# facebookresearch/detectron2

Measured on NVIDIA H100. Metric: Mask R-CNN R50-FPN training hot-path images/sec (custom-op path fwd+bwd, 2 images/GPU), higher is better.
Workload: dtype f32

## Files before the change

### detectron2_b200/csrc/deform_conv_tc.cu

```cuda
#include <algorithm>
#include <cstdlib>

#include "common.cuh"
#include "tc_common.cuh"

using namespace d2b_tc;

namespace {

constexpr int kWorkerWarps = 16;
constexpr int kWorkers = kWorkerWarps * 32;
constexpr int kThreads = kWorkers + 128;
constexpr int kLaunchRegs = (65536 / kThreads) & ~7;
constexpr int kWorkerRegs = 112, kSideRegs = 24;
static_assert(kWorkers * kWorkerRegs + (kThreads - kWorkers) * kSideRegs <= kThreads * kLaunchRegs,
              "register budget exceeds the launch allocation");
constexpr int kMaxBN = 128;
constexpr int kRowsPerHalf = 128 / (2 * kWorkerWarps);
constexpr int kTile = 16384;
constexpr int kMaxSmem = 227 * 1024;
constexpr int kGcolPitch = 132;

struct TC {
  int N, Cin, H, W, Cout, kh, kw, sh, sw, ph, pw, dh, dw, G, DG, Ho, Wo, cpg, opg, cpdg, KK, HoWo;
  int pack, SG, cps, ops, cbs, U;
  int tiles_img;
  int stages_img;
  int MC;
  int nks;
  long long off_bs, mask_bs;
  int mask_sigmoid;
};

struct Epi {
  const float* scale;
  const float* shift;
  int relu;
};

struct K1P { int BN, noct, nkp, ksplit, S, tap_bytes, stage_bytes, red; };
struct K2P { int mper, msplit, tap_bytes; };
struct K3P { int BN, noct, sper, nsplit, S, stage_bytes; };

inline size_t align256(size_t v) { return (v + 255) & ~(size_t)255; }

bool make_tc(const d2b_dcn_params* p, TC& d) {
  if (!p) return false;
  d.N = p->N; d.Cin = p->Cin; d.H = p->H; d.W = p->W; d.Cout = p->Cout; d.kh = p->kh; d.kw = p->kw;
  d.sh = p->stride_h; d.sw = p->stride_w; d.ph = p->pad_h; d.pw = p->pad_w; d.dh = p->dil_h; d.dw = p->dil_w;
  d.G = p->groups; d.DG = p->deformable_groups;
  if (d.N < 0 || d.Cin <= 0 || d.H <= 0 || d.W <= 0 || d.Cout <= 0 || d.kh <= 0 || d.kw <= 0 || d.sh <= 0 || d.sw <= 0 ||
      d.ph < 0 || d.pw < 0 || d.dh <= 0 || d.dw <= 0 || d.G <= 0 || d.DG <= 0)
    return false;
  if (d.Cin % d.G || d.Cout % d.G || d.Cin % d.DG) return false;
  d.Ho = (d.H + 2 * d.ph - (d.dh * (d.kh - 1) + 1)) / d.sh + 1;
  d.Wo = (d.W + 2 * d.pw - (d.dw * (d.kw - 1) + 1)) / d.sw + 1;
  if (d.Ho <= 0 || d.Wo <= 0) return false;
  d.cpg = d.Cin / d.G; d.opg = d.Cout / d.G; d.cpdg = d.Cin / d.DG; d.KK = d.kh * d.kw; d.HoWo = d.Ho * d.Wo;
  if (d.cpg >= 64) {
    if (d.cpg % 64) return false;
    d.pack = 1;
  } else {
    if (d.cpg != 16 && d.cpg != 32) return false;
    d.pack = 64 / d.cpg;
    if (d.G % d.pack) return false;
  }
  if (d.cpdg % 64) return false;
  d.SG = d.G / d.pack; d.cps = d.cpg * d.pack; d.ops = d.opg * d.pack; d.cbs = d.cps / 64; d.U = d.KK * d.cbs;
  if (d.ops % 16) return false;
  if (d.KK > 49) return false;
  if ((long long)d.H * d.W * d.Cin >= (1LL << 29)) return false;
  if ((long long)d.HoWo * d.Cout >= (1LL << 31) || (long long)d.Cout * d.cpg * d.KK >= (1LL << 31)) return false;
  d.tiles_img = d2b_cdiv(d.HoWo, 128);
  d.stages_img = d2b_cdiv(d.HoWo, 64);
  d.MC = (d.U + 1) / 2;
  d.nks = d.ops / 64;
  if ((long long)d.N * d.tiles_img > 0x7fffffffLL) return false;
  d.off_bs = (long long)d.DG * 2 * d.KK * d.HoWo;
  d.mask_bs = (long long)d.DG * d.KK * d.HoWo;
  d.mask_sigmoid = 0;
  return true;
}

const float* use_fused_offset_mask(TC& d, const float* offset_mask) {
  d.off_bs = d.mask_bs = (long long)d.DG * 3 * d.KK * d.HoWo;
  d.mask_sigmoid = 1;
  return offset_mask + (size_t)d.DG * 2 * d.KK * d.HoWo;
}

int largest_tile(int n) {
  for (int t = kMaxBN; t >= 16; t >>= 1)
    if (n % t == 0) return t;
  return 0;
}

int best_split(long long base, int work, int max_split, int overhead) {
  int best = 1;
  long long best_cost = -1;
  for (int s = 1; s <= max_split; ++s) {
    const int per = d2b_cdiv(work, s);
    const int parts = d2b_cdiv(work, per);
    const long long cost = (long long)d2b_cdiv(base * parts, d2b_num_sms()) * (per + overhead);
    if (best_cost < 0 || cost < best_cost) {
      best_cost = cost;
      best = parts;
    }
  }
  return best;
}

bool plan_k1(const TC& d, K1P& k) {
  k.BN = largest_tile(d.ops);
  if (k.BN < 16) return false;
  k.noct = d.ops / k.BN;
  const int base = d.N * d.tiles_img * d.SG * k.noct;
  k.ksplit = best_split(base, d.KK, d.KK, 1);
  k.nkp = d2b_cdiv(d.KK, k.ksplit);
  k.ksplit = d2b_cdiv(d.KK, k.nkp);
  k.red = k.ksplit > 1;
  const int ndg = d.DG == 1 ? 1 : std::min(d.DG, d2b_cdiv(d.cps, d.cpdg) + 1);
  k.tap_bytes = ndg * k.nkp * 128 * 16;
  k.stage_bytes = 2 * kTile + 2 * k.BN * 128;
  k.S = 3;
  while (k.S > 1 && k.S * k.stage_bytes + k.tap_bytes + 1024 + 128 > kMaxSmem) --k.S;
  return k.S >= 2;
}

bool plan_k2(const TC& d, K2P& k) {
  if (d.ops % 64) return false;
  const int base = d.N * d.tiles_img * d.SG;
  k.msplit = best_split(base, d.MC, d.MC, 1);
  k.mper = d2b_cdiv(d.MC, k.msplit);
  k.msplit = d2b_cdiv(d.MC, k.mper);
  const int nkp = std::min(d.KK, (2 * k.mper + d.cbs - 1) / d.cbs + 1);
  const int ndg = d.DG == 1 ? 1 : std::min(d.DG, d2b_cdiv(d.cps, d.cpdg) + 1);
  k.tap_bytes = ndg * nkp * 128 * 16;
  return 2 * 4 * kTile + 128 * kGcolPitch * 4 + k.tap_bytes + 1024 + 128 <= kMaxSmem;
}

bool plan_k3(const TC& d, K3P& k) {
  if (d.ops % 64) return false;
  k.BN = largest_tile(d.ops);
  k.noct = d.ops / k.BN;
  const int units = d.MC * d.SG * k.noct;
  const int total = d.N * d.stages_img;
  k.nsplit = best_split(units, total, std::min(total, 4 * d2b_num_sms()), 3);
  k.sper = d2b_cdiv(total, k.nsplit);
  k.nsplit = d2b_cdiv(total, k.sper);
  k.stage_bytes = 2 * kTile + 2 * k.BN * 128;
  k.S = 3;
  while (k.S > 1 && k.S * k.stage_bytes + 4096 + 1024 + 128 > kMaxSmem) --k.S;
  return k.S >= 2;
}

struct TapRaw {
  float oh, ow, m;
};

__device__ __forceinline__ TapRaw tap_loads(const TC& d, const float* __restrict__ offset, const float* __restrict__ mask,
                                            int b, int dg, int kp, int p) {
  TapRaw r = {0.f, 0.f, 1.f};
  if (p < d.HoWo) {
    const size_t ob = (size_t)b * d.off_bs + ((size_t)dg * 2 * d.KK) * d.HoWo;
    r.oh = __ldg(offset + ob + (size_t)(2 * kp) * d.HoWo + p);
    r.ow = __ldg(offset + ob + (size_t)(2 * kp + 1) * d.HoWo + p);
    if (mask) r.m = __ldg(mask + (size_t)b * d.mask_bs + ((size_t)dg * d.KK + kp) * d.HoWo + p);
  }
  return r;
}

__device__ __forceinline__ int4 tap_finish(const TC& d, const TapRaw& r, bool has_mask, int kp, int p) {
  int4 t = make_int4(0, 0, 0, 0);
  if (p < d.HoWo) {
    const int ho = p / d.Wo, wo = p - ho * d.Wo;
    const int ki = kp / d.kw, kj = kp - ki * d.kw;
    const float hf = (float)(ho * d.sh - d.ph + ki * d.dh) + r.oh;
    const float wf = (float)(wo * d.sw - d.pw + kj * d.dw) + r.ow;
    float m = r.m;
    if (has_mask && d.mask_sigmoid) m = 1.f / (1.f + expf(-m));
    if (hf > -1.f && wf > -1.f && hf < (float)d.H && wf < (float)d.W) {
      const float hfl = floorf(hf), wfl = floorf(wf);
      const int hl = (int)hfl, wl = (int)wfl;
      const bool t0 = hl >= 0, t1 = hl + 1 <= d.H - 1, l0 = wl >= 0, l1 = wl + 1 <= d.W - 1;
      const int flags = (t0 && l0 ? 1 : 0) | (t0 && l1 ? 2 : 0) | (t1 && l0 ? 4 : 0) | (t1 && l1 ? 8 : 0);
      t.x = ((hl * d.W + wl + d.W + 1) << 4) | flags;
      t.y = __float_as_int(hf - hfl);
      t.z = __float_as_int(wf - wfl);
      t.w = __float_as_int(m);
    }
  }
  return t;
}

__device__ __forceinline__ int4 make_tap(const TC& d, const float* __restrict__ offset, const float* __restrict__ mask,
                                         int b, int dg, int kp, int p) {
  return tap_finish(d, tap_loads(d, offset, mask, b, dg, kp, p), mask != nullptr, kp, p);
}

struct Taps4 {
  float4 v0, v1, v2, v3;
};

__device__ __forceinline__ void load_corners(const float* __restrict__ xcb, uint32_t Cin, uint32_t rs, int code, Taps4& t) {
  const float* __restrict__ p = xcb + (uint32_t)(code >> 4) * Cin;
  const float4 z = make_float4(0.f, 0.f, 0.f, 0.f);
  t.v0 = (code & 1) ? __ldg(reinterpret_cast<const float4*>(p)) : z;
  t.v1 = (code & 2) ? __ldg(reinterpret_cast<const float4*>(p + Cin)) : z;
  t.v2 = (code & 4) ? __ldg(reinterpret_cast<const float4*>(p + rs)) : z;
  t.v3 = (code & 8) ? __ldg(reinterpret_cast<const float4*>(p + (rs + Cin))) : z;
}

__device__ __forceinline__ void interp4(const Taps4& t, float w0, float w1, float w2, float w3, float (&v)[4]) {
  const F2 z = f2_pack(0.f, 0.f), p0 = f2_pack(w0, w0), p1 = f2_pack(w1, w1), p2 = f2_pack(w2, w2), p3 = f2_pack(w3, w3);
  F2 a = f2_fma(p0, f2_pack(t.v0.x, t.v0.y), z), b = f2_fma(p0, f2_pack(t.v0.z, t.v0.w), z);
  a = f2_fma(p1, f2_pack(t.v1.x, t.v1.y), a);
  b = f2_fma(p1, f2_pack(t.v1.z, t.v1.w), b);
  a = f2_fma(p2, f2_pack(t.v2.x, t.v2.y), a);
  b = f2_fma(p2, f2_pack(t.v2.z, t.v2.w), b);
  a = f2_fma(p3, f2_pack(t.v3.x, t.v3.y), a);
  b = f2_fma(p3, f2_pack(t.v3.z, t.v3.w), b);
  f2_unpack(a, v[0], v[1]);
  f2_unpack(b, v[2], v[3]);
}

__device__ __forceinline__ void gather_store(const Taps4& t, int4 tap, uint8_t* a_hi, uint8_t* a_lo, uint32_t off,
                                             bool split) {
  const float lh = __int_as_float(tap.y), lw = __int_as_float(tap.z), m = __int_as_float(tap.w);
  const float hh = 1.f - lh, hw = 1.f - lw;
  float v[4];
  interp4(t, hh * hw * m, hh * lw * m, lh * hw * m, lh * lw * m, v);
  uint2 hi, lo;
  split4(v, hi, lo);
  *reinterpret_cast<uint2*>(a_hi + off) = hi;
  if (split) *reinterpret_cast<uint2*>(a_lo + off) = lo;
}

template <int BN, int kTransA, int kSplit>
__device__ __forceinline__ void mma_stage_(float (&acc)[BN / 4], uint32_t a_hi, uint32_t a_lo, uint32_t b_hi, uint32_t b_lo) {
  const int g = (threadIdx.x >> 7);
  const uint32_t ao = kTransA ? (uint32_t)(g & 1) * 8192u : (uint32_t)(g & 1) * 64u * 128u;
  const uint32_t bo = (uint32_t)(g >> 1) * (uint32_t)(BN / 2) * 128u;
  const uint32_t lbo = kTransA ? 8192u : 0u;
  wgmma_fence();
#pragma unroll
  for (int kk = 0; kk < 4; ++kk) {
    const uint32_t ak = ao + (kTransA ? (uint32_t)kk * 2048u : (uint32_t)kk * 32u), bk = bo + (uint32_t)kk * 32u;
    Wgmma<BN / 2, kTransA>::mma(acc, wgmma_desc(a_hi + ak, lbo, 1024), wgmma_desc(b_hi + bk, 0, 1024), 1);
    if (kSplit) {
      Wgmma<BN / 2, kTransA>::mma(acc, wgmma_desc(a_hi + ak, lbo, 1024), wgmma_desc(b_lo + bk, 0, 1024), 1);
      Wgmma<BN / 2, kTransA>::mma(acc, wgmma_desc(a_lo + ak, lbo, 1024), wgmma_desc(b_hi + bk, 0, 1024), 1);
    }
  }
  wgmma_commit();
}
template <int BN, int kTransA>
__device__ __forceinline__ void mma_stage(float (&acc)[BN / 4], uint32_t a_hi, uint32_t a_lo, uint32_t b_hi, uint32_t b_lo,
                                          int split) {
  if (split) mma_stage_<BN, kTransA, 1>(acc, a_hi, a_lo, b_hi, b_lo);
  else mma_stage_<BN, kTransA, 0>(acc, a_hi, a_lo, b_hi, b_lo);
}

template <int BN>
__device__ __forceinline__ int acc_row(int i) {
  const int t = threadIdx.x & 127;
  return (threadIdx.x >> 7 & 1) * 64 + (t >> 5) * 16 + ((t & 31) >> 2) + ((i >> 1) & 1) * 8;
}
template <int BN>
__device__ __forceinline__ int acc_col(int i) {
  return (threadIdx.x >> 8) * (BN / 2) + (i >> 2) * 8 + (threadIdx.x & 3) * 2 + (i & 1);
}

template <int BN>
__global__ void __launch_bounds__(kThreads, 1) dcn_fwd_tc_kernel(const float* __restrict__ xh,
                                                                   const float* __restrict__ offset,
                                                                   const float* __restrict__ mask,
                                                                   const uint8_t* __restrict__ wt, const Epi ep, const TC d,
                                                                   const K1P k, const int split, float* __restrict__ out,
                                                                   uint8_t* __restrict__ cols) {
  extern __shared__ uint8_t smem_raw[];
  uint8_t* smem = smem_raw + ((1024u - (smem_u32(smem_raw) & 1023u)) & 1023u);
  int4* taps = reinterpret_cast<int4*>(smem + k.S * k.stage_bytes);
  uint64_t* bars = reinterpret_cast<uint64_t*>(reinterpret_cast<uint8_t*>(taps) + k.tap_bytes);
  uint64_t* full_bar = bars;
  uint64_t* empty_bar = bars + k.S;

  const int tid = threadIdx.x, warp = tid >> 5, lane = tid & 31;
  const int b = blockIdx.x / d.tiles_img, p0 = (blockIdx.x - b * d.tiles_img) * 128;
  const int sg = blockIdx.y / k.noct, oct = blockIdx.y - sg * k.noct;
  const int kp0 = blockIdx.z * k.nkp, nkp = min(d.KK, kp0 + k.nkp) - kp0;
  const int nt = nkp * d.cbs;
  const int dg0 = (sg * d.cps) / d.cpdg;
  const bool saving = cols != nullptr && oct == 0;

  if (tid == 0) {
    for (int s = 0; s < k.S; ++s) {
      mbar_init(&full_bar[s], kWorkerWarps + 1);
      mbar_init(&empty_bar[s], kWorkerWarps + (saving ? 1 : 0));
    }
    mbar_init_fence();
  }
  if (tid < kWorkers) {
    const int ndg = ((sg + 1) * d.cps - 1) / d.cpdg - dg0 + 1;
    for (int i = tid; i < ndg * nkp * 128; i += kWorkers) {
      const int row = i & 127, r = i >> 7;
      const int dgl = r / nkp, kpl = r - dgl * nkp;
      taps[i] = make_tap(d, offset, mask, b, dg0 + dgl, kp0 + kpl, p0 + row);
    }
  }
  __syncthreads();
  if (warp < kWorkerWarps) reg_alloc<kWorkerRegs>();
  else reg_dealloc<kSideRegs>();

  if (warp < kWorkerWarps) {
    const int half = lane >> 4, q = lane & 15;
    const float* __restrict__ ximg = xh + (size_t)b * d.H * d.W * d.Cin - (size_t)(d.W + 1) * d.Cin;
    const uint32_t ucin = (uint32_t)d.Cin, urs = (uint32_t)(d.W * d.Cin);
    float acc[BN / 4];
#pragma unroll
    for (int i = 0; i < BN / 4; ++i) acc[i] = 0.f;
    int kpl = 0, cb = 0;
    auto stage = [&](int t) {
      const int s = t % k.S;
      const uint32_t par = (uint32_t)((t / k.S) & 1);
      const int cbase = sg * d.cps + cb * 64;
      const int4* __restrict__ tp = taps + ((cbase / d.cpdg - dg0) * nkp + kpl) * 128;
      const float* __restrict__ xc = ximg + cbase + q * 4;
      uint8_t* a_hi = smem + s * k.stage_bytes;
      uint8_t* a_lo = a_hi + kTile;
      mbar_wait(&empty_bar[s], par ^ 1u);
      {
        int4 tap[kRowsPerHalf];
        Taps4 c[kRowsPerHalf];
#pragma unroll
        for (int j = 0; j < kRowsPerHalf; ++j) tap[j] = tp[warp * 2 * kRowsPerHalf + j * 2 + half];
#pragma unroll
        for (int j = 0; j < kRowsPerHalf; ++j) load_corners(xc, ucin, urs, tap[j].x, c[j]);
#pragma unroll
        for (int j = 0; j < kRowsPerHalf; ++j) {
          const uint32_t r = (uint32_t)(warp * 2 * kRowsPerHalf + j * 2 + half);
          gather_store(c[j], tap[j], a_hi, a_lo, swz128(r, (uint32_t)(q >> 1)) + (uint32_t)(q & 1) * 8u, split != 0);
        }
      }
      fence_proxy_async();
      __syncwarp();
      if (lane == 0) mbar_arrive(&full_bar[s]);
      mbar_wait(&full_bar[s], par);
      const uint32_t sa = smem_u32(a_hi), sb = sa + 2 * kTile;
      mma_stage<BN, 0>(acc, sa, sa + kTile, sb, sb + (uint32_t)BN * 128u, split);
      if (++cb == d.cbs) { cb = 0; ++kpl; }
    };
    stage(0);
    for (int t = 1; t < nt; ++t) {
      stage(t);
      wgmma_wait<1>();
      __syncwarp();
      if (lane == 0) mbar_arrive(&empty_bar[(t - 1) % k.S]);
    }
    wgmma_wait<0>();
    const int oc0 = sg * d.ops + oct * k.BN;
    const bool add_shift = ep.shift != nullptr && blockIdx.z == 0;
#pragma unroll
    for (int i = 0; i < BN / 4; ++i) {
      const int p = p0 + acc_row<BN>(i);
      if (p >= d.HoWo) continue;
      const int oc = oc0 + acc_col<BN>(i);
      float* dst = out + ((size_t)b * d.Cout + oc) * d.HoWo + p;
      float v = acc[i];
      if (k.red) {
        red_add(dst, v + ((add_shift && !ep.scale && !ep.relu) ? __ldg(ep.shift + oc) : 0.f));
      } else {
        if (ep.scale) v *= __ldg(ep.scale + oc);
        if (ep.shift) v += __ldg(ep.shift + oc);
        if (ep.relu) v = fmaxf(v, 0.f);
        *dst = v;
      }
    }
  } else if (warp == kWorkerWarps) {
    if (lane == 0) {
      const uint32_t bytes = (uint32_t)(split ? 2 : 1) * (uint32_t)k.BN * 128u;
      for (int t = 0; t < nt; ++t) {
        const int s = t % k.S;
        const uint32_t par = (uint32_t)((t / k.S) & 1);
        mbar_wait(&empty_bar[s], par ^ 1u);
        const size_t tile = ((size_t)(sg * k.noct + oct) * d.U + (size_t)kp0 * d.cbs + t);
        mbar_arrive_expect_tx(&full_bar[s], bytes);
        bulk_g2s(smem + s * k.stage_bytes + 2 * kTile, wt + tile * (size_t)(2 * k.BN * 128), bytes, &full_bar[s]);
      }
    }
  } else if (warp == kWorkerWarps + 1) {
    if (saving && lane == 0) {
      const uint32_t tile_bytes = (uint32_t)(split ? 2 : 1) * (uint32_t)kTile;
      for (int t = 0; t < nt; ++t) {
        const int s = t % k.S;
        const uint32_t par = (uint32_t)((t / k.S) & 1);
        mbar_wait(&full_bar[s], par);
        const size_t tile = ((size_t)blockIdx.x * d.SG + sg) * d.U + (size_t)kp0 * d.cbs + t;
        bulk_s2g(cols + tile * tile_bytes, smem + s * k.stage_bytes, tile_bytes);
        bulk_commit();
        bulk_wait_read0();
        mbar_arrive(&empty_bar[s]);
      }
      bulk_wait0();
    }
  }
}

__global__ void __launch_bounds__(kThreads, 1) dcn_bwd_data_tc_kernel(const float* __restrict__ xh,
                                                                      const float* __restrict__ offset,
                                                                      const float* __restrict__ mask,
                                                                      const uint8_t* __restrict__ gt,
                                                                      const uint8_t* __restrict__ wt, const TC d,
                                                                      const K2P k, const int split,
                                                                      float* __restrict__ gxh, float* __restrict__ goff,
                                                                      float* __restrict__ gmask) {
  extern __shared__ uint8_t smem_raw[];
  uint8_t* smem = smem_raw + ((1024u - (smem_u32(smem_raw) & 1023u)) & 1023u);
  constexpr int kStage = 4 * kTile;
  float* gcol = reinterpret_cast<float*>(smem + 2 * kStage);
  int4* taps = reinterpret_cast<int4*>(smem + 2 * kStage + 128 * kGcolPitch * 4);
  uint64_t* bars = reinterpret_cast<uint64_t*>(reinterpret_cast<uint8_t*>(taps) + k.tap_bytes);
  uint64_t* full_bar = bars;
  uint64_t* empty_bar = bars + 2;

  const int tid = threadIdx.x, warp = tid >> 5, lane = tid & 31;
  const int b = blockIdx.x / d.tiles_img, pt = blockIdx.x - b * d.tiles_img, p0 = pt * 128;
  const int sg = blockIdx.y;
  const int m0 = blockIdx.z * k.mper, m1 = min(d.MC, m0 + k.mper), nm = m1 - m0;
  const int u_begin = 2 * m0, u_end = min(d.U, 2 * m1);
  const int kp0 = u_begin / d.cbs, nkp = (u_end - 1) / d.cbs - kp0 + 1;
  const int dg0 = (sg * d.cps) / d.cpdg;

  if (tid == 0) {
    for (int s = 0; s < 2; ++s) {
      mbar_init(&full_bar[s], 1);
      mbar_init(&empty_bar[s], kWorkerWarps);
    }
    mbar_init_fence();
  }
  if (tid < kWorkers) {
    const int ndg = ((sg + 1) * d.cps - 1) / d.cpdg - dg0 + 1;
    for (int i = tid; i < ndg * nkp * 128; i += kWorkers) {
      const int row = i & 127, r = i >> 7;
      const int dgl = r / nkp, kpl = r - dgl * nkp;
      taps[i] = make_tap(d, offset, mask, b, dg0 + dgl, kp0 + kpl, p0 + row);
    }
  }
  __syncthreads();
  if (warp < kWorkerWarps) reg_alloc<kWorkerRegs>();
  else reg_dealloc<kSideRegs>();

  if (warp < kWorkerWarps) {
    const int half = lane >> 4, q = lane & 15;
    const size_t img_off = (size_t)b * d.H * d.W * d.Cin - (size_t)(d.W + 1) * d.Cin;
    const float* __restrict__ ximg = xh + img_off;
    float* __restrict__ gimg = gxh ? gxh + img_off : nullptr;
    const uint32_t ucin = (uint32_t)d.Cin, urs = (uint32_t)(d.W * d.Cin);
    constexpr int R = kRowsPerHalf;
    float sh[R], sw[R], sm[R];
#pragma unroll
    for (int j = 0; j < R; ++j) sh[j] = sw[j] = sm[j] = 0.f;
    int cur_kp = -1, cur_dg = -1;

    auto flush = [&]() {
      if (cur_kp < 0) return;
      static_assert(R == 4, "the reduction below is written for 4 rows per half-warp");
      float v12[12];
#pragma unroll
      for (int j = 0; j < R; ++j) {
        v12[3 * j] = sh[j];
        v12[3 * j + 1] = sw[j];
        v12[3 * j + 2] = sm[j];
      }
      const bool b8 = q & 8, b4 = q & 4, b2 = q & 2, b1 = q & 1;
      float v6[6], v3[3];
#pragma unroll
      for (int i = 0; i < 6; ++i) {
        const float keep = b8 ? v12[i + 6] : v12[i], send = b8 ? v12[i] : v12[i + 6];
        v6[i] = keep + __shfl_xor_sync(0xffffffffu, send, 8);
      }
#pragma unroll
      for (int i = 0; i < 3; ++i) {
        const float keep = b4 ? v6[i + 3] : v6[i], send = b4 ? v6[i] : v6[i + 3];
        v3[i] = keep + __shfl_xor_sync(0xffffffffu, send, 4);
      }
      const float k0 = b2 ? v3[2] : v3[0], s0 = b2 ? v3[0] : v3[2];
// ... 120 lines not shown
    if (lane == 0) {
      const uint32_t half_bytes = (uint32_t)(split ? 2 : 1) * (uint32_t)kTile;
      int c = 0;
      for (int ml = 0; ml < nm; ++ml) {
        const int m = m0 + ml;
        for (int ks = 0; ks < d.nks; ++ks, ++c) {
          const int s = c & 1;
          const uint32_t par = (uint32_t)((c >> 1) & 1);
          mbar_wait(&empty_bar[s], par ^ 1u);
          mbar_arrive_expect_tx(&full_bar[s], 2 * half_bytes);
          const size_t atile = (((size_t)b * d.tiles_img + pt) * d.SG + sg) * d.nks + ks;
          const size_t btile = ((size_t)sg * d.MC + m) * d.nks + ks;
          bulk_g2s(smem + s * kStage, gt + atile * (size_t)(2 * kTile), half_bytes, &full_bar[s]);
          bulk_g2s(smem + s * kStage + 2 * kTile, wt + btile * (size_t)(2 * kTile), half_bytes, &full_bar[s]);
        }
      }
    }
  }
}

template <int BN>
__device__ __forceinline__ void gw_tile_store(const float (&acc)[BN / 4], float* __restrict__ tile, int pitch) {
#pragma unroll
  for (int i = 0; i < BN / 4; i += 2) red_add_v2(tile + (size_t)acc_row<BN>(i) * pitch + acc_col<BN>(i), acc[i], acc[i + 1]);
}

__global__ void dcn_gw_reduce_kernel(const float* __restrict__ part, const TC d, float* __restrict__ gw) {
  const long long total = (long long)d.SG * d.U * 64 * d.ops;
  const long long idx = (long long)blockIdx.x * blockDim.x + threadIdx.x;
  if (idx >= total) return;
  const int ocl = (int)(idx % d.ops);
  const long long r = idx / d.ops;
  const int rowu = (int)(r % ((long long)d.U * 64)), sg = (int)(r / ((long long)d.U * 64));
  const int u = rowu >> 6, ch = rowu & 63;
  const int kp = u / d.cbs, cb = u - kp * d.cbs;
  const int ec = sg * d.cps + cb * 64 + ch, egrp = ec / d.cpg, ecin = ec - egrp * d.cpg;
  const int oc = sg * d.ops + ocl;
  if (oc / d.opg != egrp) return;
  gw[((size_t)oc * d.cpg + ecin) * d.KK + kp] = __ldg(part + ((size_t)sg * d.MC * 128 + rowu) * d.ops + ocl);
}

constexpr int kRedOc = 16, kRedCh = 16;
__global__ void __launch_bounds__(256) dcn_gw_reduce_tile_kernel(const float* __restrict__ part, const TC d,
                                                                  float* __restrict__ gw) {
  __shared__ float tile[9 * kRedCh][kRedOc + 1];
  const int per_sg = d.cps / kRedCh;
  const int sg = blockIdx.x / per_sg, c0 = (blockIdx.x - sg * per_sg) * kRedCh;
  const int cb = c0 >> 6, ch0 = c0 & 63;
  const int ocl0 = blockIdx.y * kRedOc;
  const int tid = threadIdx.x;
  {
    const int j = tid & (kRedOc - 1), r0 = tid / kRedOc;
    for (int row = r0; row < d.KK * kRedCh; row += 256 / kRedOc) {
      const int kp = row / kRedCh, ch = row - kp * kRedCh;
      tile[row][j] = __ldg(part + ((size_t)sg * d.MC * 128 + (size_t)(kp * d.cbs + cb) * 64 + ch0 + ch) * d.ops + ocl0 + j);
    }
  }
  __syncthreads();
  const int ec0 = sg * d.cps + c0;
  for (int i = tid; i < kRedOc * kRedCh * d.KK; i += 256) {
    const int j = i / (kRedCh * d.KK), e = i - j * (kRedCh * d.KK);
    const int ch = e / d.KK, kp = e - ch * d.KK;
    const int oc = sg * d.ops + ocl0 + j, grp = oc / d.opg;
    const int ec = ec0 + ch;
    if (ec / d.cpg == grp) gw[((size_t)oc * d.cpg + (ec - grp * d.cpg)) * d.KK + kp] = tile[kp * kRedCh + ch][j];
  }
}

template <int BN>
__global__ void __launch_bounds__(kThreads, 1) dcn_bwd_weight_tc_kernel(const float* __restrict__ xh,
                                                                        const float* __restrict__ offset,
                                                                        const float* __restrict__ mask,
                                                                        const uint8_t* __restrict__ gt, const TC d,
                                                                        const K3P k, const int split,
                                                                        float* __restrict__ gw) {
  extern __shared__ uint8_t smem_raw[];
  uint8_t* smem = smem_raw + ((1024u - (smem_u32(smem_raw) & 1023u)) & 1023u);
  int4* tap_s = reinterpret_cast<int4*>(smem + k.S * k.stage_bytes);
  uint64_t* bars = reinterpret_cast<uint64_t*>(reinterpret_cast<uint8_t*>(tap_s) + 4096);
  uint64_t* full_bar = bars;
  uint64_t* empty_bar = bars + k.S;

  const int tid = threadIdx.x, warp = tid >> 5, lane = tid & 31;
  const int mb = blockIdx.x;
  const int sg = blockIdx.z / k.noct, oct = blockIdx.z - sg * k.noct;
  const int total = d.N * d.stages_img;
  const int gs0 = blockIdx.y * k.sper, gs1 = min(total, gs0 + k.sper), ns = gs1 - gs0;

  if (tid == 0) {
    for (int s = 0; s < k.S; ++s) {
      mbar_init(&full_bar[s], kWorkerWarps + 1);
      mbar_init(&empty_bar[s], kWorkerWarps);
    }
    mbar_init_fence();
  }
  __syncthreads();
  if (warp < kWorkerWarps) reg_alloc<kWorkerRegs>();
  else reg_dealloc<kSideRegs>();

  if (warp < kWorkerWarps) {
    const int half = lane >> 4, q = lane & 15;
    const int u = 2 * mb + half;
    const bool u_ok = u < d.U;
    const int kp = u_ok ? u / d.cbs : 0, cb = u_ok ? u - kp * d.cbs : 0;
    const int cbase = sg * d.cps + cb * 64;
    const int dg = cbase / d.cpdg;
    constexpr int PX = 64 / kWorkerWarps;
    const int tl_half = (lane / PX) & 1, tl_j = lane % PX;
    const int tl_u = 2 * mb + tl_half;
    const bool tl_ok = lane < 2 * PX && tl_u < d.U;
    const int tl_kp = tl_ok ? tl_u / d.cbs : 0;
    const int tl_dg = tl_ok ? (sg * d.cps + (tl_u - tl_kp * d.cbs) * 64) / d.cpdg : 0;
    int4* my_taps = tap_s + warp * 2 * (2 * PX);
    auto stage_of = [&](int i, int& b, int& pbase) {
      const int gs = gs0 + i;
      b = gs / d.stages_img;
      pbase = (gs - b * d.stages_img) * 64;
    };
    if (ns > 0) {
      int b0, pb0;
      stage_of(0, b0, pb0);
      if (lane < 2 * PX) my_taps[lane] = tl_ok ? make_tap(d, offset, mask, b0, tl_dg, tl_kp, pb0 + warp * PX + tl_j) : make_int4(0, 0, 0, 0);
    }
    __syncwarp();
    float acc[BN / 4];
#pragma unroll
    for (int i = 0; i < BN / 4; ++i) acc[i] = 0.f;
    auto stage = [&](int i) {
      const int s = i % k.S;
      const uint32_t par = (uint32_t)((i / k.S) & 1);
      int b, pbase, bn = 0, pbn = 0;
      stage_of(i, b, pbase);
      const bool have_next = i + 1 < ns;
      TapRaw raw = {0.f, 0.f, 1.f};
      if (have_next) {
        stage_of(i + 1, bn, pbn);
        if (tl_ok) raw = tap_loads(d, offset, mask, bn, tl_dg, tl_kp, pbn + warp * PX + tl_j);
      }
      const float* __restrict__ xc = xh + ((size_t)b * d.H * d.W - (size_t)(d.W + 1)) * d.Cin + cbase + q * 4;
      const uint32_t ucin = (uint32_t)d.Cin, urs = (uint32_t)(d.W * d.Cin);
      uint8_t* a_hi = smem + s * k.stage_bytes + half * 8192;
      uint8_t* a_lo = a_hi + kTile;
      const int4* cur = my_taps + (i & 1) * (2 * PX) + half * PX;
      mbar_wait(&empty_bar[s], par ^ 1u);
      {
        int4 tap[PX];
        Taps4 c[PX];
#pragma unroll
        for (int j = 0; j < PX; ++j) tap[j] = cur[j];
#pragma unroll
        for (int j = 0; j < PX; ++j) load_corners(xc, ucin, urs, tap[j].x, c[j]);
#pragma unroll
        for (int j = 0; j < PX; ++j) {
          const uint32_t r = (uint32_t)(warp * PX + j);
          gather_store(c[j], tap[j], a_hi, a_lo, swz128(r, (uint32_t)(q >> 1)) + (uint32_t)(q & 1) * 8u, split != 0);
        }
      }
      if (have_next && lane < 2 * PX)
        my_taps[((i + 1) & 1) * (2 * PX) + lane] =
            tl_ok ? tap_finish(d, raw, mask != nullptr, tl_kp, pbn + warp * PX + tl_j) : make_int4(0, 0, 0, 0);
      fence_proxy_async();
      __syncwarp();
      if (lane == 0) mbar_arrive(&full_bar[s]);
      mbar_wait(&full_bar[s], par);
      const uint32_t sa = smem_u32(smem + s * k.stage_bytes), sb = sa + 2 * kTile;
      mma_stage<BN, 1>(acc, sa, sa + kTile, sb, sb + (uint32_t)BN * 128u, split);
    };
    stage(0);
    for (int i = 1; i < ns; ++i) {
      stage(i);
      wgmma_wait<1>();
      __syncwarp();
      if (lane == 0) mbar_arrive(&empty_bar[(i - 1) % k.S]);
    }
    wgmma_wait<0>();
    gw_tile_store<BN>(acc, gw + ((size_t)sg * d.MC * 128 + (size_t)mb * 128) * d.ops + (size_t)oct * k.BN, d.ops);
  } else if (warp == kWorkerWarps) {
    if (lane == 0) {
      const uint32_t bytes = (uint32_t)(split ? 2 : 1) * (uint32_t)k.BN * 128u;
      for (int i = 0; i < ns; ++i) {
        const int s = i % k.S;
        const uint32_t par = (uint32_t)((i / k.S) & 1);
        mbar_wait(&empty_bar[s], par ^ 1u);
        mbar_arrive_expect_tx(&full_bar[s], bytes);
        const size_t tile = ((size_t)(gs0 + i) * d.SG + sg) * k.noct + oct;
        bulk_g2s(smem + s * k.stage_bytes + 2 * kTile, gt + tile * (size_t)(2 * k.BN * 128), bytes, &full_bar[s]);
      }
    }
  }
}

template <int BN>
__global__ void __launch_bounds__(kThreads, 1) dcn_bwd_weight_cols_kernel(const uint8_t* __restrict__ cols,
                                                                          const uint8_t* __restrict__ gt, const TC d,
                                                                          const K3P k, const int S, const int split,
                                                                          float* __restrict__ gw) {
  extern __shared__ uint8_t smem_raw[];
  uint8_t* smem = smem_raw + ((1024u - (smem_u32(smem_raw) & 1023u)) & 1023u);
  uint64_t* bars = reinterpret_cast<uint64_t*>(smem + S * k.stage_bytes);
  uint64_t* full_bar = bars;
  uint64_t* empty_bar = bars + S;

  const int tid = threadIdx.x, warp = tid >> 5, lane = tid & 31;
  const int mb = blockIdx.x;
  const int sg = blockIdx.z / k.noct, oct = blockIdx.z - sg * k.noct;
  const int total = d.N * d.stages_img;
  const int gs0 = blockIdx.y * k.sper, gs1 = min(total, gs0 + k.sper), ns = gs1 - gs0;
  const int nu = (2 * mb + 1 < d.U) ? 2 : 1;

  if (tid == 0) {
    for (int s = 0; s < S; ++s) {
      mbar_init(&full_bar[s], 1);
      mbar_init(&empty_bar[s], kWorkerWarps);
    }
    mbar_init_fence();
  }
  if (nu == 1 && tid < kWorkers) {
    for (int s = 0; s < S; ++s)
      for (int i = tid; i < 2 * 512; i += kWorkers) {
        const int part = i >> 9, w = i & 511;
        reinterpret_cast<uint4*>(smem + s * k.stage_bytes + part * kTile + 8192)[w] = make_uint4(0, 0, 0, 0);
      }
    fence_proxy_async();
  }
  __syncthreads();
  if (warp < kWorkerWarps) reg_alloc<kWorkerRegs>();
  else reg_dealloc<kSideRegs>();

  if (warp < kWorkerWarps) {
    float acc[BN / 4];
#pragma unroll
    for (int i = 0; i < BN / 4; ++i) acc[i] = 0.f;
    auto issue = [&](int i) {
      const int s = i % S;
      mbar_wait(&full_bar[s], (uint32_t)((i / S) & 1));
      const uint32_t sa = smem_u32(smem + s * k.stage_bytes), sb = sa + 2 * kTile;
      mma_stage<BN, 1>(acc, sa, sa + kTile, sb, sb + (uint32_t)BN * 128u, split);
    };
    issue(0);
    for (int i = 1; i < ns; ++i) {
      issue(i);
      wgmma_wait<1>();
      __syncwarp();
      if (lane == 0) mbar_arrive(&empty_bar[(i - 1) % S]);
    }
    wgmma_wait<0>();
    gw_tile_store<BN>(acc, gw + ((size_t)sg * d.MC * 128 + (size_t)mb * 128) * d.ops + (size_t)oct * k.BN, d.ops);
  } else if (warp == kWorkerWarps) {
    if (lane == 0) {
      const uint32_t parts = split ? 2u : 1u;
      const uint32_t tile_bytes = parts * (uint32_t)kTile;
      const uint32_t gbytes = parts * (uint32_t)k.BN * 128u;
      for (int i = 0; i < ns; ++i) {
        const int s = i % S;
        const uint32_t par = (uint32_t)((i / S) & 1);
        const int gs = gs0 + i;
        const int b = gs / d.stages_img, st = gs - b * d.stages_img;
        mbar_wait(&empty_bar[s], par ^ 1u);
        mbar_arrive_expect_tx(&full_bar[s], (uint32_t)nu * parts * 8192u + gbytes);
        uint8_t* stage = smem + s * k.stage_bytes;
        const uint8_t* src =
            cols + ((((size_t)b * d.tiles_img + (st >> 1)) * d.SG + sg) * d.U + 2 * mb) * tile_bytes + (size_t)(st & 1) * 8192;
        for (int ul = 0; ul < nu; ++ul)
          for (uint32_t part = 0; part < parts; ++part)
            bulk_g2s(stage + part * kTile + ul * 8192, src + (size_t)ul * tile_bytes + (size_t)part * kTile, 8192u, &full_bar[s]);
        const size_t tile = ((size_t)gs * d.SG + sg) * k.noct + oct;
        bulk_g2s(stage + 2 * kTile, gt + tile * (size_t)(2 * k.BN * 128), gbytes, &full_bar[s]);
      }
    }
  }
}

__device__ __forceinline__ void split8(const float (&v)[8], uint4& hi, uint4& lo) {
  split2(v[0], v[1], hi.x, lo.x);
  split2(v[2], v[3], hi.y, lo.y);
  split2(v[4], v[5], hi.z, lo.z);
  split2(v[6], v[7], hi.w, lo.w);
}

__device__ __forceinline__ float w_elem(const float* __restrict__ w, const TC& d, int oc, int c, int kp) {
  const int g = c / d.cpg;
  if (oc / d.opg != g) return 0.f;
  return __ldg(w + ((size_t)oc * d.cpg + (c - g * d.cpg)) * d.KK + kp);
}

__global__ void dcn_wtile_fwd_kernel(const float* __restrict__ w, const TC d, int BN, int noct, uint8_t* __restrict__ dst) {
  const long long idx = (long long)blockIdx.x * blockDim.x + threadIdx.x;
  const long long total = (long long)d.SG * noct * d.U * BN * 8;
  if (idx >= total) return;
  const int c16 = (int)(idx & 7);
// ... 151 lines not shown
  if (i >= total) return;
  const int oc = (int)((i / HoWo) % Cout);
  float v = y[i];
  if (ep.scale) v *= __ldg(ep.scale + oc);
  if (ep.shift) v += __ldg(ep.shift + oc);
  if (ep.relu) v = fmaxf(v, 0.f);
  y[i] = v;
}

int to_nhwc(const float* x, const TC& d, float* dst, cudaStream_t stream) {
  d2b_pyramid P = {};
  P.num_levels = 1;
  P.feat[0] = x;
  P.H[0] = d.H;
  P.W[0] = d.W;
  P.scale[0] = 1.f;
  float* dsts[1] = {dst};
  return d2b_pyramid_nchw_to_nhwc(&P, d.N, d.Cin, dsts, (void*)stream);
}

}

int d2b_deform_conv_tc_supported(const d2b_dcn_params* p) {
  TC d;
  K1P k1;
  return make_tc(p, d) && plan_k1(d, k1);
}

int d2b_deform_conv_tc_bwd_supported(const d2b_dcn_params* p) {
  TC d;
  K2P k2;
  K3P k3;
  return make_tc(p, d) && plan_k2(d, k2) && plan_k3(d, k3);
}

size_t d2b_deform_conv_tc_fwd_workspace(const d2b_dcn_params* p, int x_nhwc) {
  TC d;
  K1P k;
  if (!make_tc(p, d) || !plan_k1(d, k)) return 0;
  size_t b = align256((size_t)d.SG * k.noct * d.U * 2 * k.BN * 128);
  if (!x_nhwc) b += align256(sizeof(float) * (size_t)d.N * d.H * d.W * d.Cin);
  return b;
}

size_t d2b_deform_conv_tc_cols_bytes(const d2b_dcn_params* p, int precision) {
  TC d;
  K1P k;
  if (precision == 0 || !make_tc(p, d) || !plan_k1(d, k)) return 0;
  return (size_t)d.N * d.tiles_img * d.SG * d.U * (size_t)(precision == 1 ? 2 : 1) * kTile;
}

int d2b_deform_conv_forward_tc(const float* x, const float* offset, const float* mask, const float* weight,
                               const float* scale, const float* shift, int relu, const d2b_dcn_params* p, int precision,
                               int tcflags, float* out, void* cols, void* workspace, size_t workspace_bytes, void* stream_) {
  cudaStream_t stream = (cudaStream_t)stream_;
  const int x_nhwc = tcflags & 1;
  TC d;
  K1P k;
  if (!make_tc(p, d) || !plan_k1(d, k)) return D2B_EUNSUPPORTED;
  if (d.N == 0) return D2B_OK;
  if (tcflags & 2) {
    if (mask) return D2B_EINVAL;
    mask = use_fused_offset_mask(d, offset);
  }
  if (!workspace || workspace_bytes < d2b_deform_conv_tc_fwd_workspace(p, x_nhwc)) return D2B_EWORKSPACE;
  if ((reinterpret_cast<uintptr_t>(workspace) & 255) || (x_nhwc && (reinterpret_cast<uintptr_t>(x) & 15)) ||
      (reinterpret_cast<uintptr_t>(cols) & 15))
    return D2B_EINVAL;
  uint8_t* ws = reinterpret_cast<uint8_t*>(workspace);
  uint8_t* wt = ws;
  ws += align256((size_t)d.SG * k.noct * d.U * 2 * k.BN * 128);
  const float* xh = x;
  if (!x_nhwc) {
    float* xn = reinterpret_cast<float*>(ws);
    int rc = to_nhwc(x, d, xn, stream);
    if (rc) return rc;
    xh = xn;
  }
  {
    const long long total = (long long)d.SG * k.noct * d.U * k.BN * 8;
    dcn_wtile_fwd_kernel<<<d2b_cdiv(total, 256), 256, 0, stream>>>(weight, d, k.BN, k.noct, wt);
    D2B_CHECK_LAUNCH();
  }
  if (k.red) D2B_CUDA(cudaMemsetAsync(out, 0, sizeof(float) * (size_t)d.N * d.Cout * d.HoWo, stream));
  const int smem_bytes = k.S * k.stage_bytes + k.tap_bytes + 1024 + 128;
  const int split = precision == 1 ? 1 : 0;
  const Epi ep = {scale, shift, relu};
  dim3 grid(d.N * d.tiles_img, d.SG * k.noct, k.ksplit);
#define D2B_LAUNCH_K1(BN)                                                                                              \
  {                                                                                                                    \
    D2B_ALLOW_BIG_SMEM(dcn_fwd_tc_kernel<BN>);                                                                         \
    dcn_fwd_tc_kernel<BN><<<grid, kThreads, smem_bytes, stream>>>(xh, offset, mask, wt, ep, d, k, split, out,        \
                                                                    reinterpret_cast<uint8_t*>(cols));                 \
  }
  if (k.BN == 16) D2B_LAUNCH_K1(16)
  else if (k.BN == 32) D2B_LAUNCH_K1(32)
  else if (k.BN == 64) D2B_LAUNCH_K1(64)
  else D2B_LAUNCH_K1(128)
#undef D2B_LAUNCH_K1
  D2B_CHECK_LAUNCH();
  if (k.red && (scale || relu)) {
    const long long total = (long long)d.N * d.Cout * d.HoWo;
    dcn_epilogue_kernel<<<d2b_cdiv(total, 256), 256, 0, stream>>>(out, total, d.Cout, d.HoWo, ep);
    D2B_CHECK_LAUNCH();
  }
  return D2B_OK;
}

size_t d2b_deform_conv_tc_bwd_workspace(const d2b_dcn_params* p, int x_nhwc, int need_data, int need_weight) {
  TC d;
  K2P k2;
  K3P k3;
  if (!make_tc(p, d) || !plan_k2(d, k2) || !plan_k3(d, k3)) return 0;
  size_t b = 0;
  const size_t xbytes = align256(sizeof(float) * (size_t)d.N * d.H * d.W * d.Cin);
  if (!x_nhwc) b += xbytes;
  if (need_data && !x_nhwc) b += xbytes;
  if (need_data) {
    b += align256((size_t)d.N * d.tiles_img * d.SG * d.nks * 2 * kTile);
    b += align256((size_t)d.SG * d.MC * d.nks * 2 * kTile);
  }
  if (need_weight) {
    b += align256((size_t)d.N * d.stages_img * d.SG * k3.noct * 2 * k3.BN * 128);
    b += align256(sizeof(float) * (size_t)d.SG * d.MC * 128 * d.ops);
  }
  return b;
}

int d2b_deform_conv_backward_tc(const float* x, const float* offset, const float* mask, const float* weight,
                                const float* grad_out, const float* scale, const float* y_saved, int relu,
                                const d2b_dcn_params* p, int precision, int tcflags, const void* cols, float* grad_x,
                                float* grad_offset, float* grad_mask, float* grad_weight, void* workspace,
                                size_t workspace_bytes, void* stream_) {
  cudaStream_t stream = (cudaStream_t)stream_;
  const int x_nhwc = tcflags & 1;
  TC d;
  K2P k2;
  K3P k3;
  if (!make_tc(p, d) || !plan_k2(d, k2) || !plan_k3(d, k3)) return D2B_EUNSUPPORTED;
  const int need_data = (grad_x || grad_offset || grad_mask) ? 1 : 0, need_weight = grad_weight ? 1 : 0;
  const bool fused_om = (tcflags & 2) != 0;
  if (fused_om && (mask || grad_mask)) return D2B_EINVAL;
  if (relu && !y_saved) return D2B_EINVAL;
  const size_t nx = (size_t)d.N * d.H * d.W * d.Cin, noff = (size_t)d.N * d.DG * (fused_om ? 3 : 2) * d.KK * d.HoWo;
  const size_t nm = (size_t)d.N * d.DG * d.KK * d.HoWo, nw = (size_t)d.Cout * d.cpg * d.KK;
  if (fused_om) {
    mask = use_fused_offset_mask(d, offset);
    if (grad_offset) grad_mask = grad_offset + (size_t)d.DG * 2 * d.KK * d.HoWo;
  }
  const Epi ep = {scale, nullptr, relu};
  if (d.N == 0 || (!need_data && !need_weight)) {
    void* zp[3] = {grad_offset, fused_om ? nullptr : grad_mask, grad_weight};
    size_t zb[3] = {noff * 4, nm * 4, nw * 4};
    return d2b_zero_buffers(zp, zb, 3, stream);
  }
  if (!workspace || workspace_bytes < d2b_deform_conv_tc_bwd_workspace(p, x_nhwc, need_data, need_weight)) return D2B_EWORKSPACE;
  if ((reinterpret_cast<uintptr_t>(workspace) & 255) || (x_nhwc && (reinterpret_cast<uintptr_t>(x) & 15)) ||
      (x_nhwc && grad_x && (reinterpret_cast<uintptr_t>(grad_x) & 15)) || (reinterpret_cast<uintptr_t>(cols) & 15))
    return D2B_EINVAL;
  const int split = precision == 1 ? 1 : 0;
  uint8_t* ws = reinterpret_cast<uint8_t*>(workspace);
  const size_t xbytes = align256(sizeof(float) * nx);
  const float* xh = x;
  if (!x_nhwc) {
    float* xn = reinterpret_cast<float*>(ws);
    ws += xbytes;
    int rc = to_nhwc(x, d, xn, stream);
    if (rc) return rc;
    xh = xn;
  }
  float* gxh = nullptr;
  if (need_data && grad_x) gxh = x_nhwc ? grad_x : reinterpret_cast<float*>(ws);
  uint8_t* gt_px = nullptr;
  uint8_t* wt = nullptr;
  if (need_data) {
    if (!x_nhwc) ws += xbytes;
    gt_px = ws;
    ws += align256((size_t)d.N * d.tiles_img * d.SG * d.nks * 2 * kTile);
    wt = ws;
    ws += align256((size_t)d.SG * d.MC * d.nks * 2 * kTile);
  }
  uint8_t* gt_oc = need_weight ? ws : nullptr;
  float* gw_part = nullptr;
  if (need_weight) {
    ws += align256((size_t)d.N * d.stages_img * d.SG * k3.noct * 2 * k3.BN * 128);
    gw_part = reinterpret_cast<float*>(ws);
  }
  {
    void* zp[4] = {grad_offset, fused_om ? nullptr : grad_mask, gxh, gw_part};
    size_t zb[4] = {noff * 4, nm * 4, nx * 4, sizeof(float) * (size_t)d.SG * d.MC * 128 * d.ops};
    int rc = d2b_zero_buffers(zp, zb, 4, stream);
    if (rc) return rc;
  }
  if (need_data) {
    dcn_gout_px_tiles_kernel<<<dim3((unsigned)((size_t)d.N * d.tiles_img * d.SG * d.nks), 4), 256, 0, stream>>>(
        grad_out, y_saved, ep, d, gt_px, gt_oc, k3.BN, k3.noct);
    D2B_CHECK_LAUNCH();
    {
      const long long total = (long long)d.SG * d.MC * d.nks * 128 * 8;
      dcn_wtile_bwd_kernel<<<d2b_cdiv(total, 256), 256, 0, stream>>>(weight, d, wt);
      D2B_CHECK_LAUNCH();
    }
    const int smem_bytes = 2 * 4 * kTile + 128 * kGcolPitch * 4 + k2.tap_bytes + 1024 + 128;
    D2B_ALLOW_BIG_SMEM(dcn_bwd_data_tc_kernel);
    dim3 grid(d.N * d.tiles_img, d.SG, k2.msplit);
    dcn_bwd_data_tc_kernel<<<grid, kThreads, smem_bytes, stream>>>(xh, offset, mask, gt_px, wt, d, k2, split, gxh, grad_offset,
                                                                  mask ? grad_mask : nullptr);
    D2B_CHECK_LAUNCH();
    if (grad_x && !x_nhwc) {
      dim3 g2(d2b_cdiv(d.H * d.W, 64), d2b_cdiv(d.Cin, 32), d.N);
      nhwc_to_nchw_kernel<<<g2, 256, 0, stream>>>(gxh, d.Cin, d.H * d.W, grad_x);
      D2B_CHECK_LAUNCH();
    }
  }
  if (need_weight) {
    if (!need_data) {
      const long long total = (long long)d.N * d.stages_img * d.SG * k3.noct * k3.BN * 8;
      dcn_gout_oc_tiles_kernel<<<d2b_cdiv(total, 256), 256, 0, stream>>>(grad_out, y_saved, ep, d, k3.BN, k3.noct, gt_oc);
      D2B_CHECK_LAUNCH();
    }
    dim3 grid(d.MC, k3.nsplit, d.SG * k3.noct);
    if (cols) {
      const int S = std::min(6, (kMaxSmem - 2048) / k3.stage_bytes);
      const int smem_bytes = S * k3.stage_bytes + 1024 + 128;
      const uint8_t* cl = reinterpret_cast<const uint8_t*>(cols);
#define D2B_LAUNCH_K3C(BN)                                                                                             \
  {                                                                                                                      \
    D2B_ALLOW_BIG_SMEM(dcn_bwd_weight_cols_kernel<BN>);                                                                \
    dcn_bwd_weight_cols_kernel<BN><<<grid, kThreads, smem_bytes, stream>>>(cl, gt_oc, d, k3, S, split, gw_part);       \
  }
      if (k3.BN == 64) D2B_LAUNCH_K3C(64)
      else D2B_LAUNCH_K3C(128)
#undef D2B_LAUNCH_K3C
    } else {
      const int smem_bytes = k3.S * k3.stage_bytes + 4096 + 1024 + 128;
#define D2B_LAUNCH_K3(BN)                                                                                              \
  {                                                                                                                      \
    D2B_ALLOW_BIG_SMEM(dcn_bwd_weight_tc_kernel<BN>);                                                                  \
    dcn_bwd_weight_tc_kernel<BN><<<grid, kThreads, smem_bytes, stream>>>(xh, offset, mask, gt_oc, d, k3, split, gw_part); \
  }
      if (k3.BN == 64) D2B_LAUNCH_K3(64)
      else D2B_LAUNCH_K3(128)
#undef D2B_LAUNCH_K3
    }
    D2B_CHECK_LAUNCH();
    {
      if (d.KK <= 9) {
        dcn_gw_reduce_tile_kernel<<<dim3(d.SG * (d.cps / kRedCh), d.ops / kRedOc), 256, 0, stream>>>(gw_part, d, grad_weight);
      } else {
        const long long total = (long long)d.SG * d.U * 64 * d.ops;
        dcn_gw_reduce_kernel<<<d2b_cdiv(total, 256), 256, 0, stream>>>(gw_part, d, grad_weight);
      }
      D2B_CHECK_LAUNCH();
    }
  }
  return D2B_OK;
}
```

Measured before the change: 243.3.

## Feed remaining forward output-channel tiles from saved im2col columns

```diff
diff --git a/detectron2_b200/csrc/deform_conv_tc.cu b/detectron2_b200/csrc/deform_conv_tc.cu
--- a/detectron2_b200/csrc/deform_conv_tc.cu
+++ b/detectron2_b200/csrc/deform_conv_tc.cu
@@ -38,7 +38,7 @@
   int relu;
 };
 
-struct K1P { int BN, noct, nkp, ksplit, S, tap_bytes, stage_bytes, red; };
+struct K1P { int BN, noct, goct, nkp, ksplit, S, tap_bytes, stage_bytes, red; };
 struct K2P { int mper, msplit, tap_bytes; };
 struct K3P { int BN, noct, sper, nsplit, S, stage_bytes; };
 
@@ -109,11 +109,12 @@
   return best;
 }
 
-bool plan_k1(const TC& d, K1P& k) {
+bool plan_k1(const TC& d, K1P& k, bool colfed = false) {
   k.BN = largest_tile(d.ops);
   if (k.BN < 16) return false;
   k.noct = d.ops / k.BN;
-  const int base = d.N * d.tiles_img * d.SG * k.noct;
+  k.goct = colfed ? 1 : k.noct;
+  const int base = d.N * d.tiles_img * d.SG * k.goct;
   k.ksplit = best_split(base, d.KK, d.KK, 1);
   k.nkp = d2b_cdiv(d.KK, k.ksplit);
   k.ksplit = d2b_cdiv(d.KK, k.nkp);
@@ -124,6 +125,22 @@
   k.S = 3;
   while (k.S > 1 && k.S * k.stage_bytes + k.tap_bytes + 1024 + 128 > kMaxSmem) --k.S;
   return k.S >= 2;
+}
+
+bool plan_k1c(const TC& d, K1P& k1, K1P& kc) {
+  const long long base = (long long)d.N * d.tiles_img * d.SG * (k1.noct - 1);
+  if (k1.goct != 1 || k1.noct < 2 || (long long)d.N * d.tiles_img * (k1.noct - 1) > 0x7fffffffLL) return false;
+  kc = k1;
+  kc.goct = k1.noct - 1;
+  kc.ksplit = best_split(base, d.KK, d.KK, 1);
+  kc.nkp = d2b_cdiv(d.KK, kc.ksplit);
+  kc.ksplit = d2b_cdiv(d.KK, kc.nkp);
+  kc.tap_bytes = 0;
+  kc.S = 3;
+  while (kc.S > 1 && kc.S * kc.stage_bytes + 1024 + 128 > kMaxSmem) --kc.S;
+  if (kc.S < 2) return false;
+  k1.red = kc.red = k1.ksplit > 1 || kc.ksplit > 1;
+  return true;
 }
 
 bool plan_k2(const TC& d, K2P& k) {
@@ -271,6 +288,28 @@
 }
 
 template <int BN>
+__device__ __forceinline__ void fwd_epilogue(const float (&acc)[BN / 4], const Epi& ep, const TC& d, const K1P& k,
+                                             float* __restrict__ out, int b, int p0, int oc0) {
+  const bool add_shift = ep.shift != nullptr && blockIdx.z == 0;
+#pragma unroll
+  for (int i = 0; i < BN / 4; ++i) {
+    const int p = p0 + acc_row<BN>(i);
+    if (p >= d.HoWo) continue;
+    const int oc = oc0 + acc_col<BN>(i);
+    float* dst = out + ((size_t)b * d.Cout + oc) * d.HoWo + p;
+    float v = acc[i];
+    if (k.red) {
+      red_add(dst, v + ((add_shift && !ep.scale && !ep.relu) ? __ldg(ep.shift + oc) : 0.f));
+    } else {
+      if (ep.scale) v *= __ldg(ep.scale + oc);
+      if (ep.shift) v += __ldg(ep.shift + oc);
+      if (ep.relu) v = fmaxf(v, 0.f);
+      *dst = v;
+    }
+  }
+}
+
+template <int BN>
 __global__ void __launch_bounds__(kThreads, 1) dcn_fwd_tc_kernel(const float* __restrict__ xh,
                                                                    const float* __restrict__ offset,
                                                                    const float* __restrict__ mask,
@@ -286,7 +325,7 @@
 
   const int tid = threadIdx.x, warp = tid >> 5, lane = tid & 31;
   const int b = blockIdx.x / d.tiles_img, p0 = (blockIdx.x - b * d.tiles_img) * 128;
-  const int sg = blockIdx.y / k.noct, oct = blockIdx.y - sg * k.noct;
+  const int sg = blockIdx.y / k.goct, oct = blockIdx.y - sg * k.goct;
   const int kp0 = blockIdx.z * k.nkp, nkp = min(d.KK, kp0 + k.nkp) - kp0;
   const int nt = nkp * d.cbs;
   const int dg0 = (sg * d.cps) / d.cpdg;
@@ -357,24 +396,7 @@
       if (lane == 0) mbar_arrive(&empty_bar[(t - 1) % k.S]);
     }
     wgmma_wait<0>();
-    const int oc0 = sg * d.ops + oct * k.BN;
-    const bool add_shift = ep.shift != nullptr && blockIdx.z == 0;
-#pragma unroll
-    for (int i = 0; i < BN / 4; ++i) {
-      const int p = p0 + acc_row<BN>(i);
-      if (p >= d.HoWo) continue;
-      const int oc = oc0 + acc_col<BN>(i);
-      float* dst = out + ((size_t)b * d.Cout + oc) * d.HoWo + p;
-      float v = acc[i];
-      if (k.red) {
-        red_add(dst, v + ((add_shift && !ep.scale && !ep.relu) ? __ldg(ep.shift + oc) : 0.f));
-      } else {
-        if (ep.scale) v *= __ldg(ep.scale + oc);
-        if (ep.shift) v += __ldg(ep.shift + oc);
-        if (ep.relu) v = fmaxf(v, 0.f);
-        *dst = v;
-      }
-    }
+    fwd_epilogue<BN>(acc, ep, d, k, out, b, p0, sg * d.ops + oct * k.BN);
   } else if (warp == kWorkerWarps) {
     if (lane == 0) {
       const uint32_t bytes = (uint32_t)(split ? 2 : 1) * (uint32_t)k.BN * 128u;
@@ -401,6 +423,76 @@
         mbar_arrive(&empty_bar[s]);
       }
       bulk_wait0();
+    }
+  }
+}
+
+template <int BN>
+__global__ void __launch_bounds__(kThreads, 1) dcn_fwd_cols_kernel(const uint8_t* __restrict__ cols,
+                                                                   const uint8_t* __restrict__ wt, const Epi ep, const TC d,
+                                                                   const K1P k, const int split, float* __restrict__ out) {
+  extern __shared__ uint8_t smem_raw[];
+  uint8_t* smem = smem_raw + ((1024u - (smem_u32(smem_raw) & 1023u)) & 1023u);
+  uint64_t* bars = reinterpret_cast<uint64_t*>(smem + k.S * k.stage_bytes);
+  uint64_t* full_bar = bars;
+  uint64_t* empty_bar = bars + k.S;
+
+  const int tid = threadIdx.x, warp = tid >> 5, lane = tid & 31;
+  const int tile = blockIdx.x / k.goct, oct = 1 + (blockIdx.x - tile * k.goct);
+  const int b = tile / d.tiles_img, p0 = (tile - b * d.tiles_img) * 128;
+  const int sg = blockIdx.y;
+  const int kp0 = blockIdx.z * k.nkp, nkp = min(d.KK, kp0 + k.nkp) - kp0;
+  const int nt = nkp * d.cbs;
+
+  if (tid == 0) {
+    for (int s = 0; s < k.S; ++s) {
+      mbar_init(&full_bar[s], 1);
+      mbar_init(&empty_bar[s], kWorkerWarps);
+    }
+    mbar_init_fence();
+  }
+  __syncthreads();
+  if (warp < kWorkerWarps) reg_alloc<kWorkerRegs>();
+  else reg_dealloc<kSideRegs>();
+
+  if (warp < kWorkerWarps) {
+    float acc[BN / 4];
+#pragma unroll
+    for (int i = 0; i < BN / 4; ++i) acc[i] = 0.f;
+    auto issue = [&](int t) {
+      const int s = t % k.S;
+      mbar_wait(&full_bar[s], (uint32_t)((t / k.S) & 1));
+      const uint32_t sa = smem_u32(smem + s * k.stage_bytes), sb = sa + 2 * kTile;
+      mma_stage<BN, 0>(acc, sa, sa + kTile, sb, sb + (uint32_t)BN * 128u, split);
+    };
+    issue(0);
+    for (int t = 1; t < nt; ++t) {
+      issue(t);
+      wgmma_wait<1>();
+      __syncwarp();
+      if (lane == 0) mbar_arrive(&empty_bar[(t - 1) % k.S]);
+    }
+    wgmma_wait<0>();
+    fwd_epilogue<BN>(acc, ep, d, k, out, b, p0, sg * d.ops + oct * k.BN);
+  } else if (warp == kWorkerWarps) {
+    if (lane == 0) {
+      const uint32_t parts = split ? 2u : 1u;
+      const uint32_t abytes = parts * (uint32_t)kTile;
+      const size_t u0 = (size_t)kp0 * d.cbs;
+      const uint8_t* asrc = cols + (((size_t)tile * d.SG + sg) * d.U + u0) * abytes;
+      const uint8_t* bsrc = wt + ((size_t)(sg * k.noct + oct) * d.U + u0) * (size_t)(2 * BN * 128);
+      int s = 0;
+      uint32_t par = 1u;
+      for (int t = nt; t > 0; --t, asrc += abytes, bsrc += 2 * BN * 128) {
+        mbar_wait(&empty_bar[s], par);
+        mbar_arrive_expect_tx(&full_bar[s], abytes / 128u * (128u + BN));
+        bulk_g2s(smem + s * k.stage_bytes, asrc, abytes, &full_bar[s]);
+        bulk_g2s(smem + s * k.stage_bytes + 2 * kTile, bsrc, abytes / 128u * BN, &full_bar[s]);
+        if (++s == k.S) {
+          s = 0;
+          par ^= 1u;
+        }
+      }
     }
   }
 }
@@ -687,10 +779,10 @@
   uint64_t* empty_bar = bars + k.S;
 
   const int tid = threadIdx.x, warp = tid >> 5, lane = tid & 31;
-  const int mb = blockIdx.x;
-  const int sg = blockIdx.z / k.noct, oct = blockIdx.z - sg * k.noct;
+  const int mb = blockIdx.y;
+  const int sg = blockIdx.x / k.noct, oct = blockIdx.x - sg * k.noct;
   const int total = d.N * d.stages_img;
-  const int gs0 = blockIdx.y * k.sper, gs1 = min(total, gs0 + k.sper), ns = gs1 - gs0;
+  const int gs0 = blockIdx.z * k.sper, gs1 = min(total, gs0 + k.sper), ns = gs1 - gs0;
 
   if (tid == 0) {
     for (int s = 0; s < k.S; ++s) {
@@ -807,10 +899,10 @@
   uint64_t* empty_bar = bars + S;
 
   const int tid = threadIdx.x, warp = tid >> 5, lane = tid & 31;
-  const int mb = blockIdx.x;
-  const int sg = blockIdx.z / k.noct, oct = blockIdx.z - sg * k.noct;
+  const int mb = blockIdx.y;
+  const int sg = blockIdx.x / k.noct, oct = blockIdx.x - sg * k.noct;
   const int total = d.N * d.stages_img;
-  const int gs0 = blockIdx.y * k.sper, gs1 = min(total, gs0 + k.sper), ns = gs1 - gs0;
+  const int gs0 = blockIdx.z * k.sper, gs1 = min(total, gs0 + k.sper), ns = gs1 - gs0;
   const int nu = (2 * mb + 1 < d.U) ? 2 : 1;
 
   if (tid == 0) {
@@ -1128,11 +1220,20 @@
     dcn_wtile_fwd_kernel<<<d2b_cdiv(total, 256), 256, 0, stream>>>(weight, d, k.BN, k.noct, wt);
     D2B_CHECK_LAUNCH();
   }
+  K1P kc;
+  bool colfed = false;
+  if (cols && k.noct > 1) {
+    K1P k1;
+    if (plan_k1(d, k1, true) && plan_k1c(d, k1, kc)) {
+      k = k1;
+      colfed = true;
+    }
+  }
   if (k.red) D2B_CUDA(cudaMemsetAsync(out, 0, sizeof(float) * (size_t)d.N * d.Cout * d.HoWo, stream));
   const int smem_bytes = k.S * k.stage_bytes + k.tap_bytes + 1024 + 128;
   const int split = precision == 1 ? 1 : 0;
   const Epi ep = {scale, shift, relu};
-  dim3 grid(d.N * d.tiles_img, d.SG * k.noct, k.ksplit);
+  dim3 grid(d.N * d.tiles_img, d.SG * k.goct, k.ksplit);
 #define D2B_LAUNCH_K1(BN)                                                                                              \
   {                                                                                                                    \
     D2B_ALLOW_BIG_SMEM(dcn_fwd_tc_kernel<BN>);                                                                         \
@@ -1145,6 +1246,22 @@
   else D2B_LAUNCH_K1(128)
 #undef D2B_LAUNCH_K1
   D2B_CHECK_LAUNCH();
+  if (colfed) {
+    const int smem_c = kc.S * kc.stage_bytes + 1024 + 128;
+    dim3 grid_c(d.N * d.tiles_img * kc.goct, d.SG, kc.ksplit);
+    const uint8_t* cl = reinterpret_cast<const uint8_t*>(cols);
+#define D2B_LAUNCH_K1C(BN)                                                                                             \
+  {                                                                                                                    \
+    D2B_ALLOW_BIG_SMEM(dcn_fwd_cols_kernel<BN>);                                                                       \
+    dcn_fwd_cols_kernel<BN><<<grid_c, kThreads, smem_c, stream>>>(cl, wt, ep, d, kc, split, out);                      \
+  }
+    if (kc.BN == 16) D2B_LAUNCH_K1C(16)
+    else if (kc.BN == 32) D2B_LAUNCH_K1C(32)
+    else if (kc.BN == 64) D2B_LAUNCH_K1C(64)
+    else D2B_LAUNCH_K1C(128)
+#undef D2B_LAUNCH_K1C
+    D2B_CHECK_LAUNCH();
+  }
   if (k.red && (scale || relu)) {
     const long long total = (long long)d.N * d.Cout * d.HoWo;
     dcn_epilogue_kernel<<<d2b_cdiv(total, 256), 256, 0, stream>>>(out, total, d.Cout, d.HoWo, ep);
@@ -1265,7 +1382,7 @@
       dcn_gout_oc_tiles_kernel<<<d2b_cdiv(total, 256), 256, 0, stream>>>(grad_out, y_saved, ep, d, k3.BN, k3.noct, gt_oc);
       D2B_CHECK_LAUNCH();
     }
-    dim3 grid(d.MC, k3.nsplit, d.SG * k3.noct);
+    dim3 grid(d.SG * k3.noct, d.MC, k3.nsplit);
     if (cols) {
       const int S = std::min(6, (kMaxSmem - 2048) / k3.stage_bytes);
       const int smem_bytes = S * k3.stage_bytes + 1024 + 128;
```

After: 251.3 (median of 6 runs). 3.3% higher.
